# NorthStarUAS/ImageAnalysis

Measured on AMD Instinct MI355X. Metric: image_pairs_matched_per_sec, higher is better.
Workload: dtype u8 (int8 MFMA, int32 accumulate)

## Files before the change

### imageanalysis_amd/csrc/match_knn2sym.hip

```cpp
#include "iamx_common.h"

namespace {

typedef int v4i __attribute__((ext_vector_type(4)));
typedef int v2i __attribute__((ext_vector_type(2)));
typedef int v16i __attribute__((ext_vector_type(16)));
typedef unsigned v2u __attribute__((ext_vector_type(2)));

#ifndef IAMX_DESC_OFFSET
#define IAMX_DESC_OFFSET 128
#endif
constexpr int D = IAMX_DESC_DIM;
constexpr int CHUNK = 128;
constexpr int BIG = 0x3F000000;

struct Pack3Args {
    const void *src;
    const int64_t *src_off;
    int64_t single_n;
    const int32_t *dst_off;
    int8_t *dst;
    int32_t *sn2, *sct, *sperm, *sinv;
    int32_t *n2, *nb, *pos;
    int n_img;
};

template <typename SRC>
__device__ __forceinline__ int load_value(const SRC *p, int i)
{
    if constexpr (sizeof(SRC) == 1) {
        return (int)p[i];
    } else {
        int v = (int)rintf((float)p[i]);
        return v < 0 ? 0 : (v > 255 ? 255 : v);
    }
}

template <typename SRC>
__global__ __launch_bounds__(256) void pack3_rows_kernel(Pack3Args P, int64_t total_rows)
{
    const int64_t t = (int64_t)blockIdx.x * 256 + threadIdx.x;
    const int64_t row = t >> 3;
    const int part = (int)(t & 7);
    int s2 = 0, s1 = 0;
    if (row < total_rows) {
        const SRC *p = static_cast<const SRC *>(P.src) + row * D + part * 16;
#pragma unroll
        for (int i = 0; i < 16; ++i) {
            const int s = load_value(p, i) - IAMX_DESC_OFFSET;
            s2 += s * s;
            s1 += s;
        }
    }
#pragma unroll
    for (int m = 1; m < 8; m <<= 1) {
        s2 += __shfl_xor(s2, m, 8);
        s1 += __shfl_xor(s1, m, 8);
    }
    if (row < total_rows && part == 0) {
        P.n2[row] = s2;
        P.nb[row] = s2 + 2 * s1;
    }
}

constexpr int RANK_BINS = 4096;
constexpr int RANK_BIN_LIMIT = 1024;
constexpr int RANK_TODO = 0x52414E4B;

__global__ __launch_bounds__(1024) void pack3_rank_bins_kernel(Pack3Args P)
{
    __shared__ int start[RANK_BINS + 1];
    __shared__ int cursor[RANK_BINS];
    __shared__ int wsum[16];
    __shared__ int s_lo, s_hi, s_max;
    const int img = blockIdx.x, tid = threadIdx.x, lane = tid & 63, wave = tid >> 6;
    const int64_t r0 = P.src_off ? P.src_off[img] : 0;
    const int n = (int)(P.src_off ? P.src_off[img + 1] - r0 : P.single_n);
    const int d0 = P.dst_off ? P.dst_off[img] : 0;
    if (n <= 0) return;
    const int32_t *key = P.n2 + r0;
    int32_t *list_row = P.sperm + d0, *list_key = P.sinv + d0;
    if (tid == 0) { s_lo = 0x7FFFFFFF; s_hi = -0x7FFFFFFF; s_max = 0; }
    for (int b = tid; b < RANK_BINS; b += 1024) cursor[b] = 0;
    __syncthreads();
    int lo = 0x7FFFFFFF, hi = -0x7FFFFFFF;
    for (int r = tid; r < n; r += 1024) {
        const int k = key[r];
        lo = min(lo, k);
        hi = max(hi, k);
    }
#pragma unroll
    for (int m = 32; m >= 1; m >>= 1) {
        lo = min(lo, __shfl_xor(lo, m));
        hi = max(hi, __shfl_xor(hi, m));
    }
    if (lane == 0) { atomicMin(&s_lo, lo); atomicMax(&s_hi, hi); }
    __syncthreads();
    lo = s_lo;
    int shift = 0;
    while (((int64_t)s_hi - lo) >> shift >= RANK_BINS) ++shift;
    for (int r = tid; r < n; r += 1024) atomicAdd(&cursor[(key[r] - lo) >> shift], 1);
    __syncthreads();
    int c[4], t = 0, mx = 0;
#pragma unroll
    for (int k = 0; k < 4; ++k) {
        c[k] = cursor[4 * tid + k];
        t += c[k];
        mx = max(mx, c[k]);
    }
    int x = t;
#pragma unroll
    for (int sft = 1; sft < 64; sft <<= 1) {
        const int y = __shfl_up(x, sft);
        if (lane >= sft) x += y;
    }
    if (lane == 63) wsum[wave] = x;
#pragma unroll
    for (int m = 32; m >= 1; m >>= 1) mx = max(mx, __shfl_xor(mx, m));
    if (lane == 0) atomicMax(&s_max, mx);
    __syncthreads();
    int woff = 0;
    for (int w = 0; w < wave; ++w) woff += wsum[w];
    int run = woff + x - t;
#pragma unroll
    for (int k = 0; k < 4; ++k) {
        start[4 * tid + k] = run;
        run += c[k];
    }
    if (tid == 1023) start[RANK_BINS] = run;
    __syncthreads();
    if (s_max > RANK_BIN_LIMIT) {
        if (tid == 0) P.sct[d0] = RANK_TODO;
        return;
    }
    if (tid == 0) P.sct[d0] = 0;
    for (int b = tid; b < RANK_BINS; b += 1024) cursor[b] = start[b];
    __syncthreads();
    for (int r = tid; r < n; r += 1024) {
        const int k = key[r];
        const int at = atomicAdd(&cursor[(k - lo) >> shift], 1);
        list_row[at] = r;
        list_key[at] = k;
    }
    __threadfence_block();
    __syncthreads();
    for (int r = tid; r < n; r += 1024) {
        const int k = key[r], b = (k - lo) >> shift;
        const int e = start[b + 1];
        int cnt = start[b];
        for (int i = start[b]; i < e; ++i) {
            const int kj = list_key[i], j = list_row[i];
            cnt += (kj < k) || (kj == k && j < r);
        }
// ... 590 lines not shown
                    __syncthreads();
                    stage_direct(ch + 2 < nchunks ? ch + 2 : nchunks - 1, buf);
                    merge_rows(ch - 1, rbo_prev, merger && ch > 0);
                }
                if (st + 1 < NS) issue((st + 1) / PP, 2 * ((st + 1) % PP), accs[cur ^ 1][0], accs[cur ^ 1][1]);
                else issue(0, 0, accs[cur ^ 1][0], accs[cur ^ 1][1]);
                {
                    const int T = (st + 1) / PP + 1, i = (st + 1) % PP;
#pragma unroll
                    for (int k = i * 8 / PP; k < (i + 1) * 8 / PP; ++k)
                        load_op(T < NT4 ? buf : buf ^ 1, T % NT4, k, aop[T & 1], tbop[T & 1]);
                }
                const v16i acc0 = accs[cur][0], acc1 = accs[cur][1];
                int t0 = min(min(m[qp][t & 3], acc0[0]), acc0[1]);
                int t1m = min(min(m[qp + 1][t & 3], acc1[0]), acc1[1]);
#pragma unroll
                for (int reg = 2; reg < 16; reg += 2) {
                    t0 = min(min(t0, acc0[reg]), acc0[reg + 1]);
                    t1m = min(min(t1m, acc1[reg]), acc1[reg + 1]);
                }
                m[qp][t & 3] = t0;
                m[qp + 1][t & 3] = t1m;
                int (&rc_)[16] = r[t & 1];
                if (qp == 0) {
#pragma unroll
                    for (int reg = 0; reg < 16; ++reg) rc_[reg] = min(acc0[reg], acc1[reg]);
                } else {
#pragma unroll
                    for (int reg = 0; reg < 16; ++reg) rc_[reg] = min(min(rc_[reg], acc0[reg]), acc1[reg]);
                }
                {
                    int (&rp)[16] = r[(t + 1) & 1];
                    const int tp = t > 0 ? t - 1 : NT4 - 1;
                    int *dst = row_dst + (t > 0 ? rbo : rbo_prev) + tp * 32;
                    if constexpr (PP == 1) {
                        int m0, m1;
                        half_wave_min16<true>(rp, lo_lane, m0, m1);
                        dst[0] = m0;
                        dst[16] = m1;
                    } else {
                        if (0 * PP / 4 == st % PP) row_min16_piece<0>(rp, bu, lo_lane, dst);
                        if (1 * PP / 4 == st % PP) row_min16_piece<1>(rp, bu, lo_lane, dst);
                        if (2 * PP / 4 == st % PP) row_min16_piece<2>(rp, bu, lo_lane, dst);
                        if (3 * PP / 4 == st % PP) row_min16_piece<3>(rp, bu, lo_lane, dst);
                    }
                }
#pragma unroll
                for (int i = 0; i < 8; ++i) {
                    __builtin_amdgcn_sched_group_barrier(0x008, 1, 0);
                    __builtin_amdgcn_sched_group_barrier(0x002, PIPE, 0);
                }
                __builtin_amdgcn_sched_barrier(0);
            }
            }
            rbo_prev = rbo;
            rbo = rbo == 2 * NW * CHUNK ? 0 : rbo + NW * CHUNK;
        }
        int64_t col_v = 0;
        if constexpr (ITEMS) col_v = A.col_off[u];
        {
            int m0, m1;
            half_wave_min16<true>(r[(NT4 - 1) & 1], lo_lane, m0, m1);
            int *dst = row_dst + rbo_prev + (NT4 - 1) * 32;
            dst[0] = m0;
            dst[16] = m1;
        }
        wait_direct();
        __syncthreads();
        merge_rows(nchunks - 1, rbo_prev, merger);

        const int64_t col_u = ITEMS ? uniform64(col_v) : 0;
        if (wave_valid) {
            unsigned ownpack = 0;
            int v1s[QW], v2s[QW];
#pragma unroll
            for (int qb = 0; qb < QW; ++qb) {
                const int lo01 = min(m[qb][0], m[qb][1]), hi01 = max(m[qb][0], m[qb][1]);
                const int lo23 = min(m[qb][2], m[qb][3]), hi23 = max(m[qb][2], m[qb][3]);
                const int a1 = min(lo01, lo23), a2 = min(max(lo01, lo23), min(hi01, hi23));
                const int b1 = __shfl_xor(a1, 32), b2 = __shfl_xor(a2, 32);
                const int v1 = min(a1, b1), v2 = min(max(a1, b1), min(a2, b2));
                v1s[qb] = v1;
                v2s[qb] = v2;
#if !defined(IAMX_T_NOMASK)
                const unsigned own = (m[qb][0] <= v2 ? 1u : 0u) | (m[qb][1] <= v2 ? 2u : 0u) |
                                     (m[qb][2] <= v2 ? 4u : 0u) | (m[qb][3] <= v2 ? 8u : 0u);
                ownpack |= own << (4 * qb);
#endif
            }
            const unsigned othpack = A.colmask ? (unsigned)__shfl_xor((int)ownpack, 32) : 0u;
            const int row0 = q0 + QW * rc;
            if (g == 0) {
#pragma unroll
                for (int qb = 0; qb < QW; ++qb)
                    if (row0 + qb < nb)
                        *reinterpret_cast<v2i *>(A.col + 2 * ((ITEMS ? col_u : A.col_off[u]) + row0 + qb)) = v2i{v1s[qb], v2s[qb]};
                if (A.colmask) {
                    uint8_t *dst = A.colmask + (ITEMS ? col_u : A.col_off[u]) + row0;
                    if (QW == 8 && row0 + QW <= nb) {
                        auto spread = [](unsigned nib4) {
                            const unsigned x = (nib4 | (nib4 << 8)) & 0x00FF00FFu;
                            return (x | (x << 4)) & 0x0F0F0F0Fu;
                        };
                        const unsigned lo = spread(ownpack & 0xFFFFu) | (spread(othpack & 0xFFFFu) << 4);
                        const unsigned hi = spread(ownpack >> 16) | (spread(othpack >> 16) << 4);
                        *reinterpret_cast<v2u *>(dst) = v2u{lo, hi};
                    } else {
#pragma unroll
                        for (int qb = 0; qb < QW; ++qb)
                            if (row0 + qb < nb)
                                dst[qb] = (uint8_t)(((ownpack >> (4 * qb)) & 15u) | (((othpack >> (4 * qb)) & 15u) << 4));
                    }
                }
            }
        }
        if constexpr (!ITEMS) break;
        else if (++u == uniform32(u_end)) break;
    }
}

struct NarTask { int p, cls, item0, n; };
struct NarLayout {
    int64_t ctl, pair_base, mask, slot, items, res, tasks, total;
    int64_t item_cap, task_cap;
};
__host__ __device__ inline NarLayout narrow_layout(int64_t rows, int64_t n_pairs)
{
    NarLayout L;
    auto up = [](int64_t v) { return (v + 255) / 256 * 256; };
    L.item_cap = rows;
    L.task_cap = rows / 64 + 80 * n_pairs + 64;
    int64_t o = 0;
    L.ctl = o;        o += 256;
    L.pair_base = o;  o += up(n_pairs * 4);
    L.mask = o;       o += up(rows * 8);
    L.slot = o;       o += up(rows * 8);
    L.items = o;      o += up(L.item_cap * 8);
    L.res = o;        o += up(L.item_cap * 16);
    L.tasks = o;      o += up(L.task_cap * 16);
    L.total = o;
    return L;
}
constexpr int NAR_MIN_TRAIN = 1024;
constexpr int NAR_ITEMS = 256;

struct CandArgs {
    const int32_t *sn2, *sperm, *img_off, *img_n;
    const int32_t *pairs;
    const int32_t *osrc;
    const int32_t *wg_off;
    const int64_t *col_off, *rowp_off, *out_off;
    const int32_t *col, *rowp;
    double thresh;
    uint8_t *keep;
    int32_t *cand_cnt;
    int32_t *cand_q;
    int32_t *task_total;
    int32_t *tasks;
    int32_t *d2;
    int wg_shift;
    const uint8_t *colmask;
    int8_t *nar;
    int64_t rows_total;
    int n_pairs, wgrows;
};

__device__ __forceinline__ void symcand_rows_pair(const CandArgs &A, int p, int pos)
{
    const int qimg = A.pairs[2 * p];
    const int u = A.osrc[2 * p], role = A.osrc[2 * p + 1];
    const int soff = A.img_off[qimg], n = A.img_n[qimg];
    if (pos >= n) return;
    const int cap = (n + CHUNK - 1) / CHUNK * CHUNK;
    const int nwg = A.wg_off[u + 1] - A.wg_off[u];
    const int64_t ob = A.out_off[p];
    const int32_t *rowq = A.rowp + 2 * A.rowp_off[u];
    const int ncls = role == 0 ? 8 : nwg;
    const bool nar_ok = A.nar != nullptr && A.img_n[A.pairs[2 * p + 1]] >= NAR_MIN_TRAIN && ncls <= 64;
    const int n2 = A.sn2[soff + pos], par = n2 & 1;
    long long Lb, Ub;
    int U2 = 0x7FFFFFFF;
    if (role == 0) {
        const v2i v = *reinterpret_cast<const v2i *>(A.col + 2 * (A.col_off[u] + pos));
        const long long cq = n2 >> 1;
        Lb = 2 * (v.x + cq) + par;
        Ub = 2 * (v.y + cq) + par + 1;
    } else {
        int L = 0x7FFFFFFF, U1 = 0x7FFFFFFF;
        for (int w = 0; w < nwg; ++w) {
            int eL, e1, e2;
            unpack_row_bounds(*reinterpret_cast<const v2i *>(rowq + 2 * ((int64_t)w * cap + pos)), eL, e1, e2);
            L = min(L, eL);
            const int n1 = min(U1, e1);
            U2 = min(max(U1, e1), min(U2, e2));
            U1 = n1;
        }
        Lb = 2ll * L + par;
        Ub = 2ll * U2 + par + 1;
    }
    if (Lb < 0) Lb = 0;
    const float f0 = (float)sqrt((double)Lb);
    const float f1 = (float)sqrt((double)Ub);
    const bool k = f1 == 0.0f || (double)f0 * ((double)f0 / (double)f1) < A.thresh;
    const int orig = A.sperm[soff + pos];
    if (k) atomicOr(reinterpret_cast<unsigned *>(A.keep) + ((ob + orig) >> 5), 1u << ((ob + orig) & 31));
    if (k) A.d2[2 * (ob + orig) + 1] = (int)(Ub < 0x7FFFFFFFll ? Ub : 0x7FFFFFFFll);
    if (k && nar_ok) {
        unsigned long long mk = 0ull;
        if (role == 0) {
            mk = A.colmask[A.col_off[u] + pos];
        } else {
            for (int w = 0; w < nwg; ++w)
                if (rowq[2 * ((int64_t)w * cap + pos)] <= U2) mk |= 1ull << w;
        }
        const NarLayout NL = narrow_layout(A.rows_total, A.n_pairs);
        reinterpret_cast<unsigned long long *>(A.nar + NL.mask)[ob + orig] = mk;
    }
}

__global__ __launch_bounds__(256) void symcand_rows_kernel(CandArgs A)
{
    for (int p = blockIdx.y; p < A.n_pairs; p += gridDim.y)
#pragma unroll 1
        for (int k = 0; k < 4; ++k) symcand_rows_pair(A, p, (blockIdx.x * 4 + k) * 256 + threadIdx.x);
}

__global__ __launch_bounds__(256) void symcand_kernel(CandArgs A)
{
    __shared__ int wcnt[4];
    __shared__ int s_base;
    const int p = blockIdx.x;
    const int qimg = A.pairs[2 * p];
    const int u = A.osrc[2 * p], role = A.osrc[2 * p + 1];
    const int n = A.img_n[qimg];
    const int nwg = A.wg_off[u + 1] - A.wg_off[u];
    const int64_t ob = A.out_off[p];
    const NarLayout NL = narrow_layout(A.rows_total, A.n_pairs);
    const int ncls = role == 0 ? 8 : nwg;
    const bool nar_ok = A.nar != nullptr && A.img_n[A.pairs[2 * p + 1]] >= NAR_MIN_TRAIN && ncls <= 64;
    unsigned long long *maskv = reinterpret_cast<unsigned long long *>(A.nar + NL.mask);
    const int lane = threadIdx.x & 63, wave = threadIdx.x >> 6;
    int out = 0;
    for (int base = 0; base < n; base += 256) {
        const int i = base + threadIdx.x;
        const bool k = i < n && ((reinterpret_cast<const unsigned *>(A.keep)[(ob + i) >> 5] >> ((ob + i) & 31)) & 1u);
        const unsigned long long mask = __ballot(k);
        const int before = __popcll(mask & ((1ull << lane) - 1ull));
        if (lane == 0) wcnt[wave] = __popcll(mask);
        __syncthreads();
        int woff = 0, tot = 0;
#pragma unroll
        for (int w = 0; w < 4; ++w) {
            if (w < wave) woff += wcnt[w];
            tot += wcnt[w];
        }
        if (k) A.cand_q[ob + out + woff + before] = i;
        out += tot;
        __syncthreads();
    }
    bool narrow = nar_ok && out > 64;
    if (A.nar != nullptr) {
        __shared__ int cls_cnt[64], cls_off[65], cls_task[65], s_nb;
        int32_t *ctl = reinterpret_cast<int32_t *>(A.nar + NL.ctl);
        int32_t *pair_base = reinterpret_cast<int32_t *>(A.nar + NL.pair_base);
        v2i *slot = reinterpret_cast<v2i *>(A.nar + NL.slot);
        v2i *items = reinterpret_cast<v2i *>(A.nar + NL.items);
        NarTask *ntasks = reinterpret_cast<NarTask *>(A.nar + NL.tasks);
        if (narrow) {
            if (threadIdx.x < 64) cls_cnt[threadIdx.x] = 0;
            __syncthreads();
            int run = 0;
            for (int base = 0; base < out; base += 256) {
                const int i = base + threadIdx.x;
                unsigned long long mk = 0ull;
                if (i < out) mk = maskv[ob + A.cand_q[ob + i]];
                const int nk = __popcll(mk);
                int x = nk;
#pragma unroll
                for (int sft = 1; sft < 64; sft <<= 1) {
                    const int y = __shfl_up(x, sft);
                    if (lane >= sft) x += y;
                }
                if (lane == 63) wcnt[wave] = x;
                __syncthreads();
                int woff = 0, tot = 0;
#pragma unroll
                for (int w = 0; w < 4; ++w) {
                    if (w < wave) woff += wcnt[w];
                    tot += wcnt[w];
                }
                if (i < out) {
                    slot[ob + i] = v2i{run + woff + x - nk, nk};
                    for (unsigned long long b = mk; b; b &= b - 1) atomicAdd(&cls_cnt[__ffsll((long long)b) - 1], 1);
                }
                run += tot;
                __syncthreads();
            }
            if (threadIdx.x == 0) {
                int o = 0, nt = 0;
                for (int cidx = 0; cidx < 64; ++cidx) {
                    cls_off[cidx] = o;
                    cls_task[cidx] = nt;
                    o += cls_cnt[cidx];
                    nt += (cls_cnt[cidx] + NAR_ITEMS - 1) / NAR_ITEMS;
                }
                cls_off[64] = o;
                cls_task[64] = nt;
                const int b0 = atomicAdd(ctl + 1, run);
                bool ok = (int64_t)b0 + run <= NL.item_cap;
                int t0 = 0;
                if (ok) {
                    t0 = atomicAdd(ctl + 0, nt);
                    ok = (int64_t)t0 + nt <= NL.task_cap;
                }
                s_nb = ok ? b0 : -1;
                s_base = t0;
                pair_base[p] = ok ? b0 : -1;
            }
            __syncthreads();
            narrow = s_nb >= 0;
            if (narrow) {
                const int b0 = s_nb, t0 = s_base;
                if (threadIdx.x < 64) {
                    const int cidx = threadIdx.x, cnt_c = cls_cnt[cidx];
                    for (int t = 0; t * NAR_ITEMS < cnt_c; ++t)
                        ntasks[t0 + cls_task[cidx] + t] =
                            NarTask{p, cidx, b0 + cls_off[cidx] + t * NAR_ITEMS, min(NAR_ITEMS, cnt_c - t * NAR_ITEMS)};
                }
                __syncthreads();
                if (threadIdx.x < 64) cls_cnt[threadIdx.x] = 0;
                __syncthreads();
                for (int i = threadIdx.x; i < out; i += 256) {
                    const unsigned long long mk = maskv[ob + A.cand_q[ob + i]];
                    int sl = b0 + slot[ob + i].x;
                    for (unsigned long long b = mk; b; b &= b - 1, ++sl) {
                        const int cidx = __ffsll((long long)b) - 1;
                        const int at = atomicAdd(&cls_cnt[cidx], 1);
                        items[b0 + cls_off[cidx] + at] = v2i{i, sl};
                    }
                }
            }
            __syncthreads();
        } else if (threadIdx.x == 0) {
            pair_base[p] = -1;
        }
    }
    if (narrow) {
        if (threadIdx.x == 0) A.cand_cnt[p] = out;
        return;
    }
    const bool small = out <= 64;
    const int ntask = small ? (out > 0 ? 1 : 0) : (out + (1 << A.wg_shift) - 1) >> A.wg_shift;
    if (threadIdx.x == 0) {
        A.cand_cnt[p] = out;
        s_base = ntask ? atomicAdd(A.task_total + (small ? 0 : 1), ntask) + (small ? 0 : (int)gridDim.x) : 0;
    }
    __syncthreads();
    const int tag = small ? 0 : (A.wg_shift << 24);
    for (int t = threadIdx.x; t < ntask; t += 256)
        *reinterpret_cast<v2i *>(A.tasks + 2 * (s_base + t)) = v2i{p, t | tag};
}

struct ExactArgs {
    const int8_t *desc;
    const int32_t *norm_q;
    const int32_t *norm_t;
    const int32_t *key_t;
    int n_pairs;
    const int32_t *img_off, *img_n;
    const int32_t *pairs;
    const int64_t *out_off;
    const int32_t *cand_cnt;
    const int32_t *cand_q;
    const int32_t *task_total, *tasks;
    double thresh;
    int32_t *d2;
    int32_t *cand_t;
    double *cand_metric;
    uint8_t *cand_keep;
    int32_t *zero_div;
};

__device__ __forceinline__ int med3_key(int a, int b, int c)
{
    int r;
    asm("v_med3_i32 %0, %1, %2, %3" : "=v"(r) : "v"(a), "v"(b), "v"(c));
    return r;
}

__global__ __launch_bounds__(256) void symexact_keys_kernel(const int32_t *__restrict__ norm_t,
                                                            int64_t total_rows,
                                                            int32_t *__restrict__ key_t)
{
    for (int64_t g = (int64_t)blockIdx.x * 256 + threadIdx.x; g < total_rows;
         g += (int64_t)gridDim.x * 256)
        key_t[g] = norm_t[g] * 256 + (int)(g & 255);
}

__device__ __forceinline__ int lshl9_add(int a, int b)
{
    return (int)(((unsigned)a << 9) + (unsigned)b);
}

__device__ __forceinline__ void exact_finish(const ExactArgs &A, int p, int64_t cb, int cnt, int qoff,
                                             int q, int k, int g, int bd1, int bi1, int bd2, int bi2)
{
    const int od1 = __shfl_xor(bd1, 32), oi1 = __shfl_xor(bi1, 32);
    const int od2 = __shfl_xor(bd2, 32), oi2 = __shfl_xor(bi2, 32);
    auto less = [](int da, int ia, int db, int ib) { return da < db || (da == db && ia < ib); };
// ... 431 lines not shown
        for (int ph = 0; ph < nph; ++ph) {
            const int buf = ph & 1;
            if (ph + 1 < nph) fetch(ph + 1, pre, pre_meta);
#pragma unroll
            for (int j = 0; j < SUB; ++j) {
                const int tile = ph * SUB + j;
                if (n_sets > 0 && tile < ntiles) {
                    v4i a[4];
#pragma unroll
                    for (int s = 0; s < 4; ++s)
                        a[s] = *reinterpret_cast<const v4i *>(&s_tile[buf][(j * 32 + c) * D + 16 * ((2 * s + g) ^ ((c >> 1) & 7))]);
                    v16i cin;
#pragma unroll
                    for (int kk = 0; kk < 4; ++kk) {
                        const v4i tv = *reinterpret_cast<const v4i *>(&s_half[buf][j * 32 + 8 * kk + 4 * g]);
                        cin[4 * kk] = tv.x; cin[4 * kk + 1] = tv.y; cin[4 * kk + 2] = tv.z; cin[4 * kk + 3] = tv.w;
                    }
#pragma unroll
                    for (int h = 0; h < 2; ++h) {
                        if (h == 1 && n_sets < 2) break;
                        v16i acc = __builtin_amdgcn_mfma_i32_32x32x32_i8(a[0], bq[h][0], cin, 0, 0, 0);
#pragma unroll
                        for (int s = 1; s < 4; ++s)
                            acc = __builtin_amdgcn_mfma_i32_32x32x32_i8(a[s], bq[h][s], acc, 0, 0, 0);
                        const int t0 = min(min(acc[0], acc[1]), acc[2]), t1 = min(min(acc[3], acc[4]), acc[5]);
                        const int t2 = min(min(acc[6], acc[7]), acc[8]), t3 = min(min(acc[9], acc[10]), acc[11]);
                        const int t4 = min(min(acc[12], acc[13]), acc[14]);
                        const int lo = min(min(min(t0, t1), t2), min(min(t3, t4), acc[15]));
                        if (__ballot(lo <= hmax[h]) == 0ull) continue;
                        v4i tk[4];
#pragma unroll
                        for (int kk = 0; kk < 4; ++kk)
                            tk[kk] = *reinterpret_cast<const v4i *>(&s_pk[buf][j * 32 + 8 * kk + 4 * g]);
                        int m1 = 0x7FFFFFFF, m2 = 0x7FFFFFFF;
#pragma unroll
                        for (int reg = 0; reg < 16; ++reg) {
                            const int key = (int)(((unsigned)acc[reg] << 5) + (unsigned)tk[reg >> 2][reg & 3]);
                            m2 = med3_key(m1, m2, key);
                            m1 = min(m1, key);
                        }
                        const int d1k = m1 >> 4, d2k = m2 >> 4;
                        if (__ballot(d1k == d2k) == 0ull) {
                            const int r1 = m1 & 15;
                            const int i1k = s_idx[buf][j * 32 + 8 * (r1 >> 2) + 4 * g + (r1 & 3)];
                            if (d1k < bd1[h] || (d1k == bd1[h] && i1k < bi1[h])) {
                                bd2[h] = min(bd1[h], d2k);
                                bd1[h] = d1k;
                                bi1[h] = i1k;
                            } else {
                                bd2[h] = min(bd2[h], d1k);
                            }
                        } else {
#pragma unroll
                            for (int reg = 0; reg < 16; ++reg) {
                                const int dk = 2 * acc[reg] + ((tk[reg >> 2][reg & 3] >> 4) & 1);
                                const int ik = s_idx[buf][j * 32 + 8 * (reg >> 2) + 4 * g + (reg & 3)];
                                if (dk < bd1[h] || (dk == bd1[h] && ik < bi1[h])) {
                                    bd2[h] = bd1[h];
                                    bd1[h] = dk;
                                    bi1[h] = ik;
                                } else {
                                    bd2[h] = min(bd2[h], dk);
                                }
                            }
                        }
                    }
                }
            }
            if (ph + 1 < nph) stage(buf ^ 1, pre, pre_meta);
            __syncthreads();
        }
#pragma unroll
        for (int h = 0; h < 2; ++h) {
            const int od1 = __shfl_xor(bd1[h], 32), oi1 = __shfl_xor(bi1[h], 32), od2 = __shfl_xor(bd2[h], 32);
            int f_d, f_i, s_d;
            if (od1 < bd1[h] || (od1 == bd1[h] && oi1 < bi1[h])) {
                f_d = od1; f_i = oi1;
                s_d = min(bd1[h], od2);
            } else {
                f_d = bd1[h]; f_i = bi1[h];
                s_d = min(od1, bd2[h]);
            }
            if (g == 0 && live[h] && (h == 0 || n_sets == 2)) res[slot[h]] = v4i{f_d, f_i, s_d, 0};
        }
    }
}

__device__ __forceinline__ void narrow_finish_pair(const NarArgs &A, int p)
{
    const NarLayout NL = narrow_layout(A.rows_total, A.n_pairs);
    const int32_t *pair_base = reinterpret_cast<const int32_t *>(A.nar + NL.pair_base);
    const v2i *slot = reinterpret_cast<const v2i *>(A.nar + NL.slot);
    const v4i *res = reinterpret_cast<const v4i *>(A.nar + NL.res);
    if (p == 0 && threadIdx.x == 0) {
        int32_t *ctl = reinterpret_cast<int32_t *>(A.nar + NL.ctl);
        ctl[0] = ctl[1] = ctl[2] = 0;
    }
    const int b0 = pair_base[p];
    if (b0 < 0) return;
    const int64_t cb = A.out_off[p];
    const int cnt = A.cand_cnt[p];
    const int qoff = A.img_off[A.pairs[2 * p]];
    for (int k = threadIdx.x; k < cnt; k += 256) {
        const v2i sl = slot[cb + k];
        int f_d = NAR_D_INVALID, f_i = NAR_D_INVALID, s_d = NAR_D_INVALID;
        for (int j = 0; j < sl.y; ++j) {
            const v4i e = res[b0 + sl.x + j];
            if (e.x < f_d || (e.x == f_d && e.y < f_i)) {
                s_d = min(f_d, e.z);
                f_d = e.x;
                f_i = e.y;
            } else {
                s_d = min(s_d, e.x);
            }
        }
        const int q = A.cand_q[cb + k];
        if (f_d >= (1 << 26) || s_d >= (1 << 26)) {
            atomicAdd(A.zero_div + 1, 1);
            A.cand_t[cb + k] = 0;
            A.cand_metric[cb + k] = 0.0;
            A.cand_keep[cb + k] = 0;
            continue;
        }
        const int na = A.norm_q[qoff + q];
        const int d1 = f_d + na, d2 = s_d + na;
        *reinterpret_cast<v2i *>(A.d2w + 2 * (cb + q)) = v2i{d1, d2};
        const float f0 = (float)sqrt((double)d1);
        const float f1 = (float)sqrt((double)d2);
        double mt;
        bool ok = false;
        if (f1 == 0.0f) {
            mt = __longlong_as_double(0x7FF8000000000000LL);
            atomicAdd(A.zero_div, 1);
        } else {
            mt = (double)f0 * ((double)f0 / (double)f1);
            ok = mt < A.thresh;
        }
        A.cand_t[cb + k] = f_i;
        A.cand_metric[cb + k] = mt;
        A.cand_keep[cb + k] = ok ? 1 : 0;
    }
}

__global__ __launch_bounds__(256) void symcompact_kernel(const int64_t *cand_off,
                                                         const int32_t *cand_cnt,
                                                         const uint8_t *cand_keep,
                                                         int32_t *q, int32_t *t,
                                                         double *metric,
                                                         int32_t *surv_cnt,
                                                         int32_t *task_total, NarArgs N)
{
    __shared__ int wcnt[4];
    const int p = blockIdx.x;
    if (N.nar != nullptr) {
        narrow_finish_pair(N, p);
        __threadfence_block();
        __syncthreads();
    }
    const int64_t b = cand_off[p];
    const int cnt = cand_cnt[p];
    const int lane = threadIdx.x & 63, wave = threadIdx.x >> 6;
    int out = 0;
    for (int base = 0; base < cnt; base += 256) {
        const int i = base + threadIdx.x;
        const bool k = i < cnt && cand_keep[b + i];
        int vq = 0, vt = 0;
        double vm = 0.0;
        if (k) { vq = q[b + i]; vt = t[b + i]; vm = metric[b + i]; }
        const unsigned long long mask = __ballot(k);
        const int before = __popcll(mask & ((1ull << lane) - 1ull));
        if (lane == 0) wcnt[wave] = __popcll(mask);
        __syncthreads();
        int woff = 0, tot = 0;
#pragma unroll
        for (int w = 0; w < 4; ++w) {
            if (w < wave) woff += wcnt[w];
            tot += wcnt[w];
        }
        if (k) {
            const int64_t o = b + out + woff + before;
            q[o] = vq; t[o] = vt; metric[o] = vm;
        }
        out += tot;
        __syncthreads();
    }
    if (threadIdx.x == 0) {
        surv_cnt[p] = out;
        if (p == 0) task_total[0] = task_total[1] = 0;
    }
}

}

extern "C" int64_t iamx_desc3_rows_cap(int64_t n_rows)
{
    if (n_rows <= 0) return 0;
    return (n_rows + CHUNK - 1) / CHUNK * CHUNK;
}

extern "C" int iamx_knn2sym_rows_per_wg(int form)
{
    return form == 2 ? 1024 : (form == 1 ? 512 : (form == 0 ? 256 : 0));
}

template <typename SRC>
static int pack3_launch(Pack3Args P, int64_t total_rows, int max_rows, void *stream, const char *what)
{
    hipStream_t st = iamx::as_stream(stream);
    if (total_rows <= 0 || max_rows <= 0) return IAMX_OK;
    const int cap = (max_rows + CHUNK - 1) / CHUNK * CHUNK;
    hipLaunchKernelGGL(pack3_rows_kernel<SRC>, dim3((unsigned)((total_rows * 8 + 255) / 256)),
                       dim3(256), 0, st, P, total_rows);
    const int64_t groups = (int64_t)((max_rows + 255) / 256) * P.n_img;
    int split = 1;
    while (split < 32 && groups * split < 2048 && max_rows > 1024 * split) split *= 2;
    if (split > 1) (void)hipMemsetAsync(P.pos, 0, (size_t)total_rows * sizeof(int32_t), st);
    hipLaunchKernelGGL(pack3_rank_bins_kernel, dim3((unsigned)P.n_img), dim3(1024), 0, st, P);
    hipLaunchKernelGGL(pack3_rank_kernel,
                       dim3((unsigned)((max_rows + 255) / 256), (unsigned)P.n_img, (unsigned)split),
                       dim3(256), 0, st, P);
    hipLaunchKernelGGL(pack3_scatter_kernel<SRC>,
                       dim3((unsigned)(((int64_t)cap * 8 + 255) / 256), (unsigned)P.n_img),
                       dim3(256), 0, st, P);
    return iamx::check_launch(what);
}

template <typename SRC>
static int pack3_single(const SRC *src, int64_t n_rows, int8_t *dst, int32_t *sn2, int32_t *sct,
                        int32_t *sperm, int32_t *sinv, int32_t *scratch, void *stream,
                        const char *what)
{
    if (n_rows < 0 || n_rows > (1 << 24) || (n_rows > 0 && !src) || !dst || !sn2 || !sct || !sperm ||
        !sinv || !scratch)
        return iamx::fail(IAMX_EINVAL, "%s: null pointer or bad row count", what);
    Pack3Args P{src, nullptr, n_rows, nullptr, dst, sn2, sct, sperm, sinv,
                scratch, scratch + n_rows, scratch + 2 * n_rows, 1};
    return pack3_launch<SRC>(P, n_rows, (int)n_rows, stream, what);
}

extern "C" int iamx_desc3_pack_u8(const uint8_t *src, int64_t n_rows, int8_t *dst, int32_t *sn2,
                                  int32_t *sct, int32_t *sperm, int32_t *sinv, int32_t *scratch,
                                  void *stream)
{
    return pack3_single(src, n_rows, dst, sn2, sct, sperm, sinv, scratch, stream, "iamx_desc3_pack_u8");
}

extern "C" int iamx_desc3_pack_f32(const float *src, int64_t n_rows, int8_t *dst, int32_t *sn2,
                                   int32_t *sct, int32_t *sperm, int32_t *sinv, int32_t *scratch,
                                   void *stream)
{
    return pack3_single(src, n_rows, dst, sn2, sct, sperm, sinv, scratch, stream, "iamx_desc3_pack_f32");
}

extern "C" int iamx_desc3_pack_batch_u8(const uint8_t *src, const int64_t *src_off,
                                        const int32_t *dst_off, int n_img, int64_t total_rows,
                                        int max_rows_per_image, int8_t *dst, int32_t *sn2,
                                        int32_t *sct, int32_t *sperm, int32_t *sinv,
                                        int32_t *scratch, void *stream)
{
    IAMX_REQUIRE(src && src_off && dst_off && dst && sn2 && sct && sperm && sinv && scratch,
                 "null pointer");
    IAMX_REQUIRE(n_img > 0 && total_rows >= 0 && max_rows_per_image >= 0, "bad count");
    Pack3Args P{src, src_off, 0, dst_off, dst, sn2, sct, sperm, sinv,
                scratch, scratch + total_rows, scratch + 2 * total_rows, n_img};
    return pack3_launch<uint8_t>(P, total_rows, max_rows_per_image, stream, "iamx_desc3_pack_batch_u8");
}

#define SWEEP_FORM2 8, 4, 0, 5, 2, 0, true, 128, 1
#define SWEEP_FORM1 4, 4, 0, 6, 2, 0, true, 128, 2
#define SWEEP_FORM0 2, 4, 0, 6, 2, 0, true, 128, 2
#define SWEEP_ITEMS2 8, 4, 1, 5, 2, 0, true, 128, 1
#define SWEEP_STR2(...) #__VA_ARGS__
#define SWEEP_STR(...) SWEEP_STR2(__VA_ARGS__)

extern "C" const char *iamx_knn2sym_kernel_id(int form)
{
    switch (form) {
    case 2: return "knn2sym_kernel<" SWEEP_STR(SWEEP_ITEMS2) ">";
    case 1: return "knn2sym_kernel<" SWEEP_STR(SWEEP_FORM1) ">";
    case 0: return "knn2sym_kernel<" SWEEP_STR(SWEEP_FORM0) ">";
    default: return "";
    }
}

extern "C" int iamx_knn2sym_sweep(const int8_t *sdesc, const int32_t *sn2, const int32_t *sct,
                                  const int32_t *img_off, const int32_t *img_n,
                                  const int32_t *upairs, const int32_t *wg_off,
                                  const int64_t *col_off, const int64_t *rowp_off, int n_u,
                                  int total_wg, int form, int32_t *col, int32_t *rowp,
                                  uint8_t *colmask, void *stream)
{
    IAMX_REQUIRE(sdesc && sn2 && sct && img_off && img_n && upairs && wg_off && col_off && rowp_off &&
                     col && rowp,
                 "null pointer");
    IAMX_REQUIRE(n_u >= 0 && total_wg >= 0, "negative count");
    IAMX_REQUIRE(form >= 0 && form <= 2, "form must be 0 (256 rows), 1 (512) or 2 (1024)");
    if (n_u == 0 || total_wg == 0) return IAMX_OK;
    SymArgs a{sdesc, sn2, sct, img_off, img_n, upairs, wg_off, col_off, rowp_off, col, rowp, n_u, total_wg,
              colmask};
    const dim3 g((unsigned)total_wg);
    hipStream_t st = iamx::as_stream(stream);
    if (form == 2) hipLaunchKernelGGL((knn2sym_kernel<SWEEP_FORM2>), g, dim3(256), 0, st, a);
    else if (form == 1) hipLaunchKernelGGL((knn2sym_kernel<SWEEP_FORM1>), g, dim3(256), 0, st, a);
    else hipLaunchKernelGGL((knn2sym_kernel<SWEEP_FORM0>), g, dim3(256), 0, st, a);
    return iamx::check_launch("iamx_knn2sym_sweep");
}

extern "C" int iamx_knn2sym_sweep_items(const int8_t *sdesc, const int32_t *sn2, const int32_t *sct,
                                        const int32_t *img_off, const int32_t *img_n,
                                        const int32_t *upairs, const int32_t *items,
                                        const int64_t *col_off, const int64_t *rowp_off, int n_u,
                                        int n_items, int32_t *col, int32_t *rowp, uint8_t *colmask,
                                        void *stream)
{
    IAMX_REQUIRE(sdesc && sn2 && sct && img_off && img_n && upairs && items && col_off && rowp_off &&
                     col && rowp,
                 "null pointer");
    IAMX_REQUIRE(n_u >= 0 && n_items >= 0, "negative count");
    if (n_u == 0 || n_items == 0) return IAMX_OK;
    SymArgs a{sdesc, sn2, sct, img_off, img_n, upairs, items, col_off, rowp_off, col, rowp, n_u, n_items,
              colmask};
    hipLaunchKernelGGL((knn2sym_kernel<SWEEP_ITEMS2>), dim3((unsigned)n_items), dim3(256), 0,
                       iamx::as_stream(stream), a);
    return iamx::check_launch("iamx_knn2sym_sweep_items");
}

static bool narrow_enabled()
{
    const char *e = getenv("IAMX_EXACT_NARROW");
    return !(e && e[0] == '0');
}

extern "C" int64_t iamx_knn2sym_narrow_bytes(int64_t rows, int n_pairs)
{
    if (rows <= 0 || n_pairs <= 0) return 0;
    return narrow_layout(rows, n_pairs).total;
}

extern "C" int iamx_knn2sym_candidates(const int32_t *sn2, const int32_t *sperm,
                                       const int32_t *img_off, const int32_t *img_n,
                                       const int32_t *pairs, const int32_t *osrc,
                                       const int32_t *wg_off, const int64_t *col_off,
                                       const int64_t *rowp_off, const int64_t *out_off,
                                       const int32_t *col, const int32_t *rowp, int n_pairs,
                                       double thresh, uint8_t *keep, int32_t *cand_cnt,
                                       int32_t *cand_q, int32_t *task_total, int32_t *tasks,
                                       int32_t *d2, const uint8_t *colmask, void *nar,
                                       int64_t rows_total, int max_query_rows, int form, void *stream)
{
    IAMX_REQUIRE(sn2 && sperm && img_off && img_n && pairs && osrc && wg_off && col_off && rowp_off &&
                     out_off && col && rowp && keep && cand_cnt && cand_q && task_total && tasks && d2,
                 "null pointer");
    IAMX_REQUIRE(!nar || colmask, "narrow workspace without colmask");
    IAMX_REQUIRE(form >= 0 && form <= 2, "form must be 0, 1 or 2");
    if (n_pairs <= 0) return IAMX_OK;
    CandArgs a{sn2, sperm, img_off, img_n, pairs, osrc, wg_off, col_off, rowp_off, out_off, col, rowp,
               thresh, keep, cand_cnt, cand_q, task_total, tasks, d2, 8,
               colmask, narrow_enabled() ? static_cast<int8_t *>(nar) : nullptr, rows_total, n_pairs,
               iamx_knn2sym_rows_per_wg(form)};
    IAMX_REQUIRE(rows_total > 0 && rows_total < (1ll << 31), "rows_total = rows of all ordered pairs");
    IAMX_REQUIRE(max_query_rows > 0, "max_query_rows = rows of the largest query image");
    (void)hipMemsetAsync(keep, 0, (size_t)((rows_total + 31) / 32 * 4), iamx::as_stream(stream));
    hipLaunchKernelGGL(symcand_rows_kernel,
                       dim3((unsigned)((max_query_rows + 1023) / 1024), (unsigned)(n_pairs < 65535 ? n_pairs : 65535)),
                       dim3(256), 0, iamx::as_stream(stream), a);
    hipLaunchKernelGGL(symcand_kernel, dim3((unsigned)n_pairs), dim3(256), 0, iamx::as_stream(stream), a);
    return iamx::check_launch("iamx_knn2sym_candidates");
}

extern "C" int iamx_knn2sym_exact(const int8_t *desc, const int32_t *norm_q, const int32_t *norm_t,
                                  int32_t *key_t, int64_t total_rows,
                                  const int32_t *img_off, const int32_t *img_n, const int32_t *pairs,
                                  const int64_t *out_off, const int32_t *cand_cnt,
                                  int32_t *task_total, const int32_t *tasks, int32_t *cand_q,
                                  int n_pairs, double thresh, int32_t *d2, int32_t *cand_t,
                                  double *cand_metric, uint8_t *cand_keep, int32_t *surv_cnt,
                                  int32_t *zero_div, const int8_t *sdesc, const int32_t *sn2,
                                  const int32_t *sct, const int32_t *sperm, const int32_t *img_off3,
                                  const int32_t *osrc, void *nar, int64_t rows_total, int form,
                                  void *stream)
{
    IAMX_REQUIRE(desc && norm_q && norm_t && key_t && img_off && img_n && pairs && out_off && cand_cnt &&
                     task_total && tasks && cand_q && d2 && cand_t && cand_metric && cand_keep &&
                     surv_cnt && zero_div,
                 "null pointer");
    IAMX_REQUIRE(total_rows >= 0, "negative row count");
    if (n_pairs <= 0) return IAMX_OK;
    hipStream_t st = iamx::as_stream(stream);
    if (total_rows > 0) {
        int64_t gk = (total_rows + 255) / 256;
        hipLaunchKernelGGL(symexact_keys_kernel, dim3((unsigned)(gk > 4096 ? 4096 : gk)), dim3(256), 0, st,
                           norm_t, total_rows, key_t);
    }
    ExactArgs a{desc, norm_q, norm_t, key_t, n_pairs, img_off, img_n, pairs, out_off, cand_cnt, cand_q,
                task_total, tasks, thresh, d2, cand_t, cand_metric, cand_keep, zero_div};
    hipLaunchKernelGGL(symexact_kernel, dim3(1024), dim3(256), 0, st, a);
    const char *prune = getenv("IAMX_EXACT_PRUNE");
    if (prune && prune[0] == '0')
        hipLaunchKernelGGL((symexact_wg_kernel<false, 1>), dim3(2048), dim3(256), 0, st, a);
    else
        hipLaunchKernelGGL((symexact_wg_kernel<true, 2>), dim3(2048), dim3(256), 0, st, a);
    NarArgs nfin{};
    if (nar && narrow_enabled()) {
        if (!(sdesc && sn2 && sct && sperm && img_off3 && osrc && rows_total > 0 && form >= 0 && form <= 2))
            return iamx::fail(IAMX_EINVAL, "iamx_knn2sym_exact: narrow workspace without the sorted store");
        NarArgs na{desc, norm_q, img_off, pairs, osrc, out_off, cand_q, d2, sdesc, sn2, sct, sperm, img_off3,
                   img_n, static_cast<int8_t *>(nar), rows_total, n_pairs, iamx_knn2sym_rows_per_wg(form),
                   cand_cnt, thresh, d2, cand_t, cand_metric, cand_keep, zero_div};
        hipLaunchKernelGGL(symnarrow_kernel<3>, dim3(768), dim3(256), 0, st, na);
        nfin = na;
    }
    hipLaunchKernelGGL(symcompact_kernel, dim3((unsigned)n_pairs), dim3(256), 0, st, out_off,
                       cand_cnt, cand_keep, cand_q, cand_t, cand_metric, surv_cnt, task_total, nfin);
    return iamx::check_launch("iamx_knn2sym_exact");
}
```

Measured before the change: 601,900.

## Vectorize candidate row kernel, add sqrt-free reject, skip empty pairs

The candidate-row kernel now handles four consecutive rows per thread with vector loads. Partial-bound merging is unrolled through a template over the workgroup count. A cheap conservative squared test rejects rows before the sqrt-based keep check, and rows are counted per pair with atomics so the compaction kernels can return early for pairs with no candidates. The keep-bit compaction now scans packed 32-bit words with a wave prefix sum instead of one bit per thread, and a custom clear kernel replaces the memset while also zeroing the counts. This adds launch-order dependencies and early-exit paths that must reset downstream state correctly.

```diff
diff --git a/imageanalysis_amd/csrc/match_knn2sym.hip b/imageanalysis_amd/csrc/match_knn2sym.hip
--- a/imageanalysis_amd/csrc/match_knn2sym.hip
+++ b/imageanalysis_amd/csrc/match_knn2sym.hip
@@ -1,4 +1,5 @@
 #include "iamx_common.h"
+#include "sym_cand_rule.h"
 
 namespace {
 
@@ -895,6 +896,7 @@
     const int64_t *col_off, *rowp_off, *out_off;
     const int32_t *col, *rowp;
     double thresh;
+    double K;
     uint8_t *keep;
     int32_t *cand_cnt;
     int32_t *cand_q;
@@ -908,64 +910,133 @@
     int n_pairs, wgrows;
 };
 
-__device__ __forceinline__ void symcand_rows_pair(const CandArgs &A, int p, int pos)
-{
-    const int qimg = A.pairs[2 * p];
-    const int u = A.osrc[2 * p], role = A.osrc[2 * p + 1];
-    const int soff = A.img_off[qimg], n = A.img_n[qimg];
-    if (pos >= n) return;
-    const int cap = (n + CHUNK - 1) / CHUNK * CHUNK;
-    const int nwg = A.wg_off[u + 1] - A.wg_off[u];
-    const int64_t ob = A.out_off[p];
-    const int32_t *rowq = A.rowp + 2 * A.rowp_off[u];
+constexpr int CAND_ROWS = 4;
+
+template <int NW>
+__device__ __forceinline__ void cand_merge_partials(const int32_t *__restrict__ rowq, int64_t cap, int (&L)[CAND_ROWS],
+                                                    int (&U1)[CAND_ROWS], int (&U2)[CAND_ROWS])
+{
+    v4i e[NW][2];
+#pragma unroll
+    for (int w = 0; w < NW; ++w) {
+        e[w][0] = *reinterpret_cast<const v4i *>(rowq + 2 * (w * cap));
+        e[w][1] = *reinterpret_cast<const v4i *>(rowq + 2 * (w * cap) + 4);
+    }
+#pragma unroll
+    for (int w = 0; w < NW; ++w)
+#pragma unroll
+        for (int i = 0; i < CAND_ROWS; ++i) {
+            int eL, e1, e2;
+            unpack_row_bounds(v2i{e[w][i >> 1][2 * (i & 1)], e[w][i >> 1][2 * (i & 1) + 1]}, eL, e1, e2);
+            L[i] = min(L[i], eL);
+            const int n1 = min(U1[i], e1);
+            U2[i] = min(max(U1[i], e1), min(U2[i], e2));
+            U1[i] = n1;
+        }
+}
+
+__device__ __forceinline__ void symcand_rows_pair(const CandArgs &A, int p, int pos0)
+{
+    const int qimg = uniform32(A.pairs[2 * p]);
+    const int u = uniform32(A.osrc[2 * p]), role = uniform32(A.osrc[2 * p + 1]);
+    const int soff = uniform32(A.img_off[qimg]), n = uniform32(A.img_n[qimg]);
+    if ((int)blockIdx.x * (256 * CAND_ROWS) >= n) return;
+    const bool in = pos0 < n;
+    const int64_t cap = (n + CHUNK - 1) / CHUNK * CHUNK;
+    const int nwg = uniform32(A.wg_off[u + 1]) - uniform32(A.wg_off[u]);
+    const int64_t ob = uniform64(A.out_off[p]);
+    const int64_t cb = uniform64(A.col_off[u]);
+    const int32_t *rowq = A.rowp + 2 * uniform64(A.rowp_off[u]);
+    int U2[CAND_ROWS];
+    long long Lb[CAND_ROWS], Ub[CAND_ROWS];
+    v4i n2 = {0, 0, 0, 0};
+    if (in) n2 = *reinterpret_cast<const v4i *>(A.sn2 + soff + pos0);
+    if (role == 0) {
+        v4i c[2] = {{0, 0, 0, 0}, {0, 0, 0, 0}};
+        if (in) {
+            c[0] = *reinterpret_cast<const v4i *>(A.col + 2 * (cb + pos0));
+            c[1] = *reinterpret_cast<const v4i *>(A.col + 2 * (cb + pos0) + 4);
+        }
+#pragma unroll
+        for (int i = 0; i < CAND_ROWS; ++i) {
+            const int par = n2[i] & 1;
+            const long long cq = n2[i] >> 1;
+            U2[i] = 0x7FFFFFFF;
+            Lb[i] = 2 * (c[i >> 1][2 * (i & 1)] + cq) + par;
+            Ub[i] = 2 * (c[i >> 1][2 * (i & 1) + 1] + cq) + par + 1;
+        }
+    } else {
+        int L[CAND_ROWS], U1[CAND_ROWS];
+#pragma unroll
+        for (int i = 0; i < CAND_ROWS; ++i) L[i] = U1[i] = U2[i] = 0x7FFFFFFF;
+        if (in) {
+            const int32_t *rq = rowq + 2 * pos0;
+            switch (nwg) {
+            case 1: cand_merge_partials<1>(rq, cap, L, U1, U2); break;
+            case 2: cand_merge_partials<2>(rq, cap, L, U1, U2); break;
+            case 3: cand_merge_partials<3>(rq, cap, L, U1, U2); break;
+            case 4: cand_merge_partials<4>(rq, cap, L, U1, U2); break;
+            default: {
+                int w = 0;
+                for (; w + 4 <= nwg; w += 4) cand_merge_partials<4>(rq + 2 * (w * cap), cap, L, U1, U2);
+                for (; w < nwg; ++w) cand_merge_partials<1>(rq + 2 * (w * cap), cap, L, U1, U2);
+            }
+            }
+        }
+#pragma unroll
+        for (int i = 0; i < CAND_ROWS; ++i) {
+            const int par = n2[i] & 1;
+            Lb[i] = 2ll * L[i] + par;
+            Ub[i] = 2ll * U2[i] + par + 1;
+        }
+    }
+    unsigned kbits = 0u;
+#pragma unroll
+    for (int i = 0; i < CAND_ROWS; ++i) {
+        if (Lb[i] < 0) Lb[i] = 0;
+        if (pos0 + i < n && !sym_cand_reject(Lb[i], Ub[i], A.K) && sym_cand_keep(Lb[i], Ub[i], A.thresh))
+            kbits |= 1u << i;
+    }
+    if (kbits == 0u) return;
+    const unsigned long long holders = __ballot(1);
+    int wave_cnt = 0;
+#pragma unroll
+    for (int i = 0; i < CAND_ROWS; ++i) wave_cnt += __popcll(__ballot((kbits >> i) & 1u));
+    if ((int)(threadIdx.x & 63) == __ffsll((long long)holders) - 1) atomicAdd(A.cand_cnt + p, wave_cnt);
     const int ncls = role == 0 ? 8 : nwg;
     const bool nar_ok = A.nar != nullptr && A.img_n[A.pairs[2 * p + 1]] >= NAR_MIN_TRAIN && ncls <= 64;
-    const int n2 = A.sn2[soff + pos], par = n2 & 1;
-    long long Lb, Ub;
-    int U2 = 0x7FFFFFFF;
-    if (role == 0) {
-        const v2i v = *reinterpret_cast<const v2i *>(A.col + 2 * (A.col_off[u] + pos));
-        const long long cq = n2 >> 1;
-        Lb = 2 * (v.x + cq) + par;
-        Ub = 2 * (v.y + cq) + par + 1;
-    } else {
-        int L = 0x7FFFFFFF, U1 = 0x7FFFFFFF;
-        for (int w = 0; w < nwg; ++w) {
-            int eL, e1, e2;
-            unpack_row_bounds(*reinterpret_cast<const v2i *>(rowq + 2 * ((int64_t)w * cap + pos)), eL, e1, e2);
-            L = min(L, eL);
-            const int n1 = min(U1, e1);
-            U2 = min(max(U1, e1), min(U2, e2));
-            U1 = n1;
-        }
-        Lb = 2ll * L + par;
-        Ub = 2ll * U2 + par + 1;
-    }
-    if (Lb < 0) Lb = 0;
-    const float f0 = (float)sqrt((double)Lb);
-    const float f1 = (float)sqrt((double)Ub);
-    const bool k = f1 == 0.0f || (double)f0 * ((double)f0 / (double)f1) < A.thresh;
-    const int orig = A.sperm[soff + pos];
-    if (k) atomicOr(reinterpret_cast<unsigned *>(A.keep) + ((ob + orig) >> 5), 1u << ((ob + orig) & 31));
-    if (k) A.d2[2 * (ob + orig) + 1] = (int)(Ub < 0x7FFFFFFFll ? Ub : 0x7FFFFFFFll);
-    if (k && nar_ok) {
-        unsigned long long mk = 0ull;
-        if (role == 0) {
-            mk = A.colmask[A.col_off[u] + pos];
-        } else {
-            for (int w = 0; w < nwg; ++w)
-                if (rowq[2 * ((int64_t)w * cap + pos)] <= U2) mk |= 1ull << w;
-        }
-        const NarLayout NL = narrow_layout(A.rows_total, A.n_pairs);
-        reinterpret_cast<unsigned long long *>(A.nar + NL.mask)[ob + orig] = mk;
+#pragma unroll
+    for (int i = 0; i < CAND_ROWS; ++i) {
+        if (!((kbits >> i) & 1u)) continue;
+        const int pos = pos0 + i;
+        const int orig = A.sperm[soff + pos];
+        atomicOr(reinterpret_cast<unsigned *>(A.keep) + ((ob + orig) >> 5), 1u << ((ob + orig) & 31));
+        A.d2[2 * (ob + orig) + 1] = (int)(Ub[i] < 0x7FFFFFFFll ? Ub[i] : 0x7FFFFFFFll);
+        if (nar_ok) {
+            unsigned long long mk = 0ull;
+            if (role == 0) {
+                mk = A.colmask[cb + pos];
+            } else {
+                for (int w = 0; w < nwg; ++w)
+                    if (rowq[2 * (w * cap + pos)] <= U2[i]) mk |= 1ull << w;
+            }
+            const NarLayout NL = narrow_layout(A.rows_total, A.n_pairs);
+            reinterpret_cast<unsigned long long *>(A.nar + NL.mask)[ob + orig] = mk;
+        }
     }
 }
 
 __global__ __launch_bounds__(256) void symcand_rows_kernel(CandArgs A)
 {
     for (int p = blockIdx.y; p < A.n_pairs; p += gridDim.y)
-#pragma unroll 1
-        for (int k = 0; k < 4; ++k) symcand_rows_pair(A, p, (blockIdx.x * 4 + k) * 256 + threadIdx.x);
+        symcand_rows_pair(A, p, ((int)blockIdx.x * 256 + (int)threadIdx.x) * CAND_ROWS);
+}
+
+__global__ __launch_bounds__(256) void symcand_clear_kernel(unsigned *keep, int64_t n_words, int32_t *cand_cnt, int n_pairs)
+{
+    const int64_t stride = (int64_t)gridDim.x * 256;
+    for (int64_t i = (int64_t)blockIdx.x * 256 + threadIdx.x; i < n_words; i += stride) keep[i] = 0u;
+    for (int64_t i = (int64_t)blockIdx.x * 256 + threadIdx.x; i < n_pairs; i += stride) cand_cnt[i] = 0;
 }
 
 __global__ __launch_bounds__(256) void symcand_kernel(CandArgs A)
@@ -973,31 +1044,52 @@
     __shared__ int wcnt[4];
     __shared__ int s_base;
     const int p = blockIdx.x;
+    const NarLayout NL = narrow_layout(A.rows_total, A.n_pairs);
+    if (A.cand_cnt[p] == 0) {
+        if (threadIdx.x == 0) {
+            A.cand_cnt[p] = 0;
+            if (A.nar != nullptr) reinterpret_cast<int32_t *>(A.nar + NL.pair_base)[p] = -1;
+        }
+        return;
+    }
     const int qimg = A.pairs[2 * p];
     const int u = A.osrc[2 * p], role = A.osrc[2 * p + 1];
     const int n = A.img_n[qimg];
     const int nwg = A.wg_off[u + 1] - A.wg_off[u];
     const int64_t ob = A.out_off[p];
-    const NarLayout NL = narrow_layout(A.rows_total, A.n_pairs);
     const int ncls = role == 0 ? 8 : nwg;
     const bool nar_ok = A.nar != nullptr && A.img_n[A.pairs[2 * p + 1]] >= NAR_MIN_TRAIN && ncls <= 64;
     unsigned long long *maskv = reinterpret_cast<unsigned long long *>(A.nar + NL.mask);
     const int lane = threadIdx.x & 63, wave = threadIdx.x >> 6;
+    const unsigned *keepw = reinterpret_cast<const unsigned *>(A.keep);
+    const int64_t w_first = ob >> 5, w_last = (ob + n - 1) >> 5;
     int out = 0;
-    for (int base = 0; base < n; base += 256) {
-        const int i = base + threadIdx.x;
-        const bool k = i < n && ((reinterpret_cast<const unsigned *>(A.keep)[(ob + i) >> 5] >> ((ob + i) & 31)) & 1u);
-        const unsigned long long mask = __ballot(k);
-        const int before = __popcll(mask & ((1ull << lane) - 1ull));
-        if (lane == 0) wcnt[wave] = __popcll(mask);
+    for (int64_t wbase = w_first; wbase <= w_last; wbase += 256) {
+        const int64_t w = wbase + threadIdx.x;
+        unsigned bits = 0u;
+        if (w <= w_last) {
+            bits = keepw[w];
+            if (w == w_first) bits &= ~0u << (ob & 31);
+            if (w == w_last) bits &= ~0u >> (31 - (int)((ob + n - 1) & 31));
+        }
+        const int c = __popc(bits);
+        int x = c;
+#pragma unroll
+        for (int sft = 1; sft < 64; sft <<= 1) {
+            const int y = __shfl_up(x, sft);
+            if (lane >= sft) x += y;
+        }
+        if (lane == 63) wcnt[wave] = x;
         __syncthreads();
         int woff = 0, tot = 0;
 #pragma unroll
-        for (int w = 0; w < 4; ++w) {
-            if (w < wave) woff += wcnt[w];
-            tot += wcnt[w];
-        }
-        if (k) A.cand_q[ob + out + woff + before] = i;
+        for (int k = 0; k < 4; ++k) {
+            if (k < wave) woff += wcnt[k];
+            tot += wcnt[k];
+        }
+        int at = out + woff + x - c;
+        const int row0 = (int)((w << 5) - ob);
+        for (unsigned b = bits; b; b &= b - 1) A.cand_q[ob + at++] = row0 + __ffs((int)b) - 1;
         out += tot;
         __syncthreads();
     }
@@ -1735,6 +1827,19 @@
 {
     __shared__ int wcnt[4];
     const int p = blockIdx.x;
+    if (cand_cnt[p] == 0) {
+        if (threadIdx.x == 0) {
+            surv_cnt[p] = 0;
+            if (p == 0) {
+                task_total[0] = task_total[1] = 0;
+                if (N.nar != nullptr) {
+                    int32_t *ctl = reinterpret_cast<int32_t *>(N.nar + narrow_layout(N.rows_total, N.n_pairs).ctl);
+                    ctl[0] = ctl[1] = ctl[2] = 0;
+                }
+            }
+        }
+        return;
+    }
     if (N.nar != nullptr) {
         narrow_finish_pair(N, p);
         __threadfence_block();
@@ -1938,12 +2043,15 @@
     IAMX_REQUIRE(form >= 0 && form <= 2, "form must be 0, 1 or 2");
     if (n_pairs <= 0) return IAMX_OK;
     CandArgs a{sn2, sperm, img_off, img_n, pairs, osrc, wg_off, col_off, rowp_off, out_off, col, rowp,
-               thresh, keep, cand_cnt, cand_q, task_total, tasks, d2, 8,
+               thresh, sym_cand_K(thresh), keep, cand_cnt, cand_q, task_total, tasks, d2, 8,
                colmask, narrow_enabled() ? static_cast<int8_t *>(nar) : nullptr, rows_total, n_pairs,
                iamx_knn2sym_rows_per_wg(form)};
     IAMX_REQUIRE(rows_total > 0 && rows_total < (1ll << 31), "rows_total = rows of all ordered pairs");
     IAMX_REQUIRE(max_query_rows > 0, "max_query_rows = rows of the largest query image");
-    (void)hipMemsetAsync(keep, 0, (size_t)((rows_total + 31) / 32 * 4), iamx::as_stream(stream));
+    const int64_t keep_words = (rows_total + 31) / 32;
+    const int64_t clear_wg = (keep_words + 4095) / 4096;
+    hipLaunchKernelGGL(symcand_clear_kernel, dim3((unsigned)(clear_wg < 256 ? clear_wg : 256)), dim3(256), 0,
+                       iamx::as_stream(stream), reinterpret_cast<unsigned *>(keep), keep_words, cand_cnt, n_pairs);
     hipLaunchKernelGGL(symcand_rows_kernel,
                        dim3((unsigned)((max_query_rows + 1023) / 1024), (unsigned)(n_pairs < 65535 ? n_pairs : 65535)),
                        dim3(256), 0, iamx::as_stream(stream), a);
diff --git a/imageanalysis_amd/csrc/sym_cand_rule.h b/imageanalysis_amd/csrc/sym_cand_rule.h
--- /dev/null
+++ b/imageanalysis_amd/csrc/sym_cand_rule.h
@@ -0,0 +1,30 @@
+#pragma once
+#include <math.h>
+
+#if defined(__HIPCC__)
+#define SYM_CAND_FN __host__ __device__ inline
+#else
+#define SYM_CAND_FN inline
+#endif
+
+inline double sym_cand_K(double thresh)
+{
+    const double inf = HUGE_VAL;
+    if (!(thresh > 0.0) || !(thresh < inf)) return inf;
+    const double K = thresh * thresh * (1.0 + 0x1p-20);
+    if (!(K >= 0x1p-1022) || !(K < inf)) return inf;
+    return K;
+}
+
+SYM_CAND_FN bool sym_cand_reject(long long Lb, long long Ub, double K)
+{
+    const double l = (double)Lb;
+    return Ub > 0 && l * l >= K * (double)Ub;
+}
+
+SYM_CAND_FN bool sym_cand_keep(long long Lb, long long Ub, double thresh)
+{
+    const float f0 = (float)sqrt((double)Lb);
+    const float f1 = (float)sqrt((double)Ub);
+    return f1 == 0.0f || (double)f0 * ((double)f0 / (double)f1) < thresh;
+}
```

New measurement: 627,500, median of 6. 4.2% higher.
